# yunjinli/visual-slam

Hardware: AMD Instinct MI355X
Metric: stereo frames/sec, detect+describe (1500 feats) + stereo match, 752x480 (higher is better)
Workload: dtype u8/f32/f64; 1 GPU; synthetic 752x480 stereo, 1500 feats/frame (BASELINE configs[1]); independent streams per GPU (configs[3]); inputs_resident_in_hbm=True, distinct_stereo_pairs_per_gpu=1024, distinct_scenes_per_gpu=64, stereo_frames_per_pass_per_gpu=1024, hip_streams=2, stereo_frames_per_launch=512, num_features=1500, match=threshold 70, ratio 1.2, cross-check

## Files before the change

### include/vslam_hip.h

```cpp
#ifndef VSLAM_HIP_H
#define VSLAM_HIP_H

#include <stddef.h>
#include <stdint.h>

#ifdef __cplusplus
extern "C" {
#endif

#define VSL_OK 0
#define VSL_ERR_INVALID (-1)
#define VSL_ERR_HIP (-2)
#define VSL_ERR_NOMEM (-3)
#define VSL_ERR_CAPACITY (-4)
#define VSL_ERR_NO_DEVICE (-5)
#define VSL_ERR_IO (-6)
#define VSL_ERR_NUMERIC (-7)

typedef struct vsl_ctx vsl_ctx;


const char* vsl_version(void);
const char* vsl_last_error(const vsl_ctx* ctx);
int vsl_device_count(void);
// ... 74 lines not shown
int vsl_frames_upload(vsl_ctx* ctx, vsl_frames* f, int first, int n, const uint8_t* imgs,
                      size_t pitch, size_t img_stride);
int vsl_host_register(vsl_ctx* ctx, void* ptr, size_t bytes);
int vsl_host_unregister(vsl_ctx* ctx, void* ptr);
int vsl_frames_detect_describe(vsl_ctx* ctx, vsl_frames* f, int first, int n, int num_features,
                               int rotate_features);
int vsl_frames_resolve_ties(vsl_ctx* ctx, vsl_frames* f, int* n_resolved);
int vsl_frames_exact_fallbacks(const vsl_frames* f);
int vsl_ctx_set_tie_eps(vsl_ctx* ctx, double eps);
int vsl_ctx_set_diagnostic(vsl_ctx* ctx, const char* name, int value);
int vsl_ctx_get_diagnostic(vsl_ctx* ctx, const char* name, int* value);

int vsl_frames_match(vsl_ctx* ctx, vsl_frames* f, const int32_t* slot_pairs, int n_pairs,
                     int threshold, double dist_2_best);
int vsl_frames_download_keypoints(vsl_ctx* ctx, vsl_frames* f, int slot, int cap,
                                  double* corners_xy, double* angles, uint64_t* desc, int* n_out);
int vsl_frames_download_matches(vsl_ctx* ctx, vsl_frames* f, int pair, int cap_pairs,
                                int32_t* pairs, int* n_out);
int vsl_frames_download_counts(vsl_ctx* ctx, vsl_frames* f, int n_images, int32_t* n_keypoints,
                               int n_pairs, int32_t* n_matches);

int vsl_frames_stereo_inliers(vsl_ctx* ctx, vsl_frames* f, int first_pair, int n_pairs, int model_a, const double* intr8_a,
                              int model_b, const double* intr8_b, const double* E9, const double* R9_0_1,
                              const double* t3_0_1, double threshold, int triangulate);
int vsl_frames_download_inliers(vsl_ctx* ctx, vsl_frames* f, int pair, int cap_pairs, int32_t* pairs, double* points_c,
                                int* n_out);
int vsl_frames_download_inlier_counts(vsl_ctx* ctx, vsl_frames* f, int n_pairs, int32_t* counts);
int vsl_find_inliers_essential(vsl_ctx* ctx, int model_a, const double* intr8_a, int model_b, const double* intr8_b,
                               const double* E9, const double* kp_a_xy, int n_a, const double* kp_b_xy, int n_b,
                               const int32_t* matches, int n_matches, double threshold, const double* R9_0_1,
                               const double* t3_0_1, int32_t* pairs_out, double* points_out, int* n_out);

int vsl_frames_download_candidate_counts(vsl_ctx* ctx, vsl_frames* f, int n_images, int32_t* n_candidates);

int vsl_diag_sqrt_check(vsl_ctx* ctx, uint32_t lo_bits, uint32_t hi_bits, unsigned long long* n_mismatch);

int vsl_diag_frames_describe_at(vsl_ctx* ctx, vsl_frames* f, int first, int n, const int32_t* corners_xy,
                                const int32_t* counts, int cap, int rotate_features, int32_t* moments,
                                int32_t* tie_rec, int tie_rec_cap, int* n_ties);

int vsl_diag_frames_set_keypoints(vsl_ctx* ctx, vsl_frames* f, int first, int n, const int32_t* counts, int cap,
                                  const int32_t* corners_xy, const uint64_t* desc);

int vsl_map_create(vsl_ctx* ctx, int cap_landmarks, int cap_descriptors, vsl_map** out);
void vsl_map_destroy(vsl_map* map);
int vsl_map_append_descriptors(vsl_map* map, int n, const uint64_t* desc, int* first_index);
int vsl_map_append_descriptors_from_frame(vsl_map* map, vsl_frames* f, int slot, int n, const int32_t* feature_ids,
                                          int* first_index);
int vsl_map_set_landmarks(vsl_map* map, int n, const double* points, const int32_t* obs_start,
                          const int32_t* obs_pool_index);
int vsl_map_info(const vsl_map* map, int* n_landmarks, int* n_observation_refs, int* n_descriptors);
int vsl_map_track(vsl_map* map, vsl_frames* f, int slot, const double* pose7, int cam_model, const double* intr8, int width,
                  int height, double cam_z_threshold, double match_max_dist_2d, int feature_match_threshold,
                  double feature_match_dist_2_best, int32_t* pairs, int* n_pairs, int* n_projected);
int vsl_map_track_corners(vsl_map* map, vsl_frames* f, int slot, const double* pose7, int cam_model, const double* intr8,
                          int width, int height, double cam_z_threshold, double match_max_dist_2d, int feature_match_threshold,
                          double feature_match_dist_2_best, int32_t* pairs, int* n_pairs, int* n_projected, double* corners_xy,
                          int* n_corners);

enum { VSL_CAM_DS = 0, VSL_CAM_PINHOLE = 1, VSL_CAM_EUCM = 2, VSL_CAM_KB4 = 3 };

typedef struct vsl_ba_problem {
  int32_t n_cams;
  int32_t n_lms;
  int32_t n_obs;
  int32_t cam_model[2];
// ... 202 lines not shown
```

### visual-slam_amd/__init__.py

```python
import ctypes as C
import os
from pathlib import Path

import numpy as np

_DIR = Path(__file__).resolve().parent
_SO = _DIR / "libvslam_hip.so"
_LIB = None

u8p = C.POINTER(C.c_uint8)
i32p = C.POINTER(C.c_int32)
u32p = C.POINTER(C.c_uint32)
u64p = C.POINTER(C.c_uint64)
i64p = C.POINTER(C.c_int64)
f32p = C.POINTER(C.c_float)
f64p = C.POINTER(C.c_double)

STAGES = ["response", "select", "describe", "match", "match_finalize", "ba_linearize", "ba_schur",
          "ba_solve", "bow_transform", "bow_score", "ba_finish", "ba_step"]

SPD_PATHS = ["none", "dense_panels", "band_panels", "band_fused", "band_two_ended", "bcr", "bcr_cyclic"]

OK = 0
CAM_DS, CAM_PINHOLE, CAM_EUCM, CAM_KB4 = 0, 1, 2, 3
# ... 1070 lines not shown

    def bow_vectors(self, first, n, voc, num_features=1500, levelsup=4, db=None, cap_per_image=None, host_outputs=True):
        L, ctx = self.ctx.L, self.ctx
        n = int(n)
        cap = (2 * num_features + 512 if cap_per_image is None else int(cap_per_image)) if host_outputs else 0
        nfeat = np.zeros(max(n, 1), np.int32)
        index = np.zeros(max(n, 1), np.int32)
        for attempt in range(2):
            m = max(n * cap, 1)
            ids, vals = np.zeros(m, np.uint32), np.zeros(m, np.float64)
            fn, ff = np.zeros(m, np.uint32), np.zeros(m, np.uint32)
            nnz, fvn = np.zeros(max(n, 1), np.int32), np.zeros(max(n, 1), np.int32)
            rc = L.vsl_frames_bow_vectors(ctx.h, self.h, int(first), n, voc.h if voc is not None else None, int(num_features),
                                          int(levelsup), db.h if db is not None else None, index.ctypes.data_as(i32p), cap,
                                          ids.ctypes.data_as(u32p), vals.ctypes.data_as(f64p), nnz.ctypes.data_as(i32p),
                                          fn.ctypes.data_as(u32p), ff.ctypes.data_as(u32p), fvn.ctypes.data_as(i32p),
                                          nfeat.ctypes.data_as(i32p))
            if rc != -4 or cap == 0 or cap_per_image is not None or nfeat[:n].max(initial=0) <= cap:
                break
            cap = int(nfeat[:n].max())
        ctx._ck(rc)
        out = None
        if host_outputs:
            out = [(ids[i * cap:i * cap + nnz[i]].copy(), vals[i * cap:i * cap + nnz[i]].copy(),
                    fn[i * cap:i * cap + fvn[i]].copy(), ff[i * cap:i * cap + fvn[i]].copy()) for i in range(n)]
        return (out, index[:n].copy()) if db is not None else out

    def candidate_counts(self, n_images):
        nc = np.zeros(max(n_images, 1), np.int32)
        self.ctx._ck(self.ctx.L.vsl_frames_download_candidate_counts(self.ctx.h, self.h, int(n_images),
                                                                     nc.ctypes.data_as(i32p)))
        return nc[:n_images].copy()

    def counts(self, n_images, n_pairs):
        nk = np.zeros(max(n_images, 1), np.int32)
        nm = np.zeros(max(n_pairs, 1), np.int32)
        self.ctx._ck(self.ctx.L.vsl_frames_download_counts(self.ctx.h, self.h, int(n_images),
                                                           nk.ctypes.data_as(i32p), int(n_pairs),
                                                           nm.ctypes.data_as(i32p)))
        return nk[:n_images].copy(), nm[:n_pairs].copy()


class Map:

    def __init__(self, ctx, cap_landmarks=4096, cap_descriptors=16384):
        self.ctx = ctx
        hnd = C.c_void_p()
        ctx._ck(ctx.L.vsl_map_create(ctx.h, int(cap_landmarks), int(cap_descriptors), C.byref(hnd)))
        self.h = hnd

    def close(self):
        if getattr(self, "h", None):
            self.ctx.L.vsl_map_destroy(self.h)
            self.h = None

    def __del__(self):
        try:
            self.close()
        except Exception:
            pass

    def append_descriptors(self, desc):
        desc = np.ascontiguousarray(desc, np.uint64).reshape(-1, 4)
        first = C.c_int32()
        self.ctx._ck(self.ctx.L.vsl_map_append_descriptors(self.h, len(desc), desc.ctypes.data_as(u64p), C.byref(first)))
        return first.value
# ... 41 lines not shown
```

### visual-slam_amd/csrc/ctx.hip

```cpp
#include <cmath>

#include "vsl_common.h"

static thread_local char g_noctx_err[512] = "";

int vsl_fail(vsl_ctx* ctx, int code, const char* fmt, ...) {
  char* dst = ctx ? ctx->err : g_noctx_err;
  va_list ap;
  va_start(ap, fmt);
  vsnprintf(dst, 512, fmt, ap);
  va_end(ap);
  return code;
}

extern "C" const char* vsl_version(void) { return "vslam_hip 0.1 (gfx950)"; }

extern "C" const char* vsl_last_error(const vsl_ctx* ctx) { return ctx ? ctx->err : g_noctx_err; }

extern "C" int vsl_device_count(void) {
  int n = 0;
  if (hipGetDeviceCount(&n) != hipSuccess) return 0;
  return n;
}

// ... 376 lines not shown
    int rc = vsl_frames_alloc(ctx, 2, w, h, feat, 1, &ctx->scratch);
    if (rc) return rc;
    ctx->scratch_w = w;
    ctx->scratch_h = h;
    ctx->scratch_feat = feat;
  }
  *out = ctx->scratch;
  return VSL_OK;
}

extern "C" int vsl_frames_download_counts(vsl_ctx* ctx, vsl_frames* f, int n_images, int32_t* n_keypoints,
                                          int n_pairs, int32_t* n_matches) {
  if (!ctx || !f || n_images < 0 || n_images > f->max_images || n_pairs < 0 || n_pairs > f->max_pairs)
    return vsl_fail(ctx, VSL_ERR_INVALID, "vsl_frames_download_counts: bad arguments");
  if (n_images > 0 && n_keypoints)
    VSL_HIP(ctx, hipMemcpyAsync(n_keypoints, f->kp_count, sizeof(int32_t) * n_images, hipMemcpyDeviceToHost, ctx->stream));
  if (n_pairs > 0 && n_matches)
    VSL_HIP(ctx, hipMemcpyAsync(n_matches, f->match_count, sizeof(int32_t) * n_pairs, hipMemcpyDeviceToHost, ctx->stream));
  VSL_HIP(ctx, hipStreamSynchronize(ctx->stream));
  return VSL_OK;
}

extern "C" int vsl_frames_download_candidate_counts(vsl_ctx* ctx, vsl_frames* f, int n_images, int32_t* n_candidates) {
  if (!ctx || !f || n_images < 0 || n_images > f->max_images || !n_candidates)
    return vsl_fail(ctx, VSL_ERR_INVALID, "vsl_frames_download_candidate_counts: bad arguments");
  if (n_images == 0) return VSL_OK;
  std::vector<int32_t> m((size_t)n_images * VSL_META_STRIDE);
  VSL_HIP(ctx, hipMemcpyAsync(m.data(), f->meta, sizeof(int32_t) * m.size(), hipMemcpyDeviceToHost, ctx->stream));
  VSL_HIP(ctx, hipStreamSynchronize(ctx->stream));
  for (int i = 0; i < n_images; i++) n_candidates[i] = m[(size_t)i * VSL_META_STRIDE + VSL_META_NCAND_LAST];
  return VSL_OK;
}

extern "C" int vsl_frames_download_keypoints(vsl_ctx* ctx, vsl_frames* f, int slot, int cap, double* corners_xy,
                                             double* angles, uint64_t* desc, int* n_out) {
  if (!ctx || !f || slot < 0 || slot >= f->max_images || !n_out || cap < 0)
    return vsl_fail(ctx, VSL_ERR_INVALID, "vsl_frames_download_keypoints: bad arguments");
  const size_t F = (size_t)f->F;
  void* hp = nullptr;
  int rc = vsl_ctx_hpinned(ctx, 64 + F * (8 + 8 + 32), &hp);
  if (rc) return rc;
  int32_t* hdr = (int32_t*)hp;
  int32_t* hxy = (int32_t*)((char*)hp + 64);
  int32_t* hmom = hxy + 2 * F;
  uint64_t* hdesc = (uint64_t*)(hmom + 2 * F);
  const size_t base = (size_t)slot * F;
  const bool ties = f->ties_pending;
  hdr[0] = 0;
  if (ties) VSL_HIP(ctx, hipMemcpyAsync(&hdr[0], f->tie_count, sizeof(int32_t), hipMemcpyDeviceToHost, ctx->stream));
  VSL_HIP(ctx, hipMemcpyAsync(&hdr[1], f->kp_count + slot, sizeof(int32_t), hipMemcpyDeviceToHost, ctx->stream));
  VSL_HIP(ctx, hipMemcpyAsync(hxy, f->kp_xy + base * 2, sizeof(int32_t) * 2 * F, hipMemcpyDeviceToHost, ctx->stream));
  if (angles) VSL_HIP(ctx, hipMemcpyAsync(hmom, f->kp_moments + base * 2, sizeof(int32_t) * 2 * F, hipMemcpyDeviceToHost, ctx->stream));
  if (desc) VSL_HIP(ctx, hipMemcpyAsync(hdesc, f->kp_desc + base * 4, sizeof(uint64_t) * 4 * F, hipMemcpyDeviceToHost, ctx->stream));
  VSL_HIP(ctx, hipStreamSynchronize(ctx->stream));
  if (ties) {
    if (hdr[0] != 0) {
      if ((rc = vsl_resolve_ties(ctx, f, nullptr))) return rc;
      if (desc) {
        VSL_HIP(ctx, hipMemcpyAsync(hdesc, f->kp_desc + base * 4, sizeof(uint64_t) * 4 * F, hipMemcpyDeviceToHost, ctx->stream));
        VSL_HIP(ctx, hipStreamSynchronize(ctx->stream));
      }
    } else {
      f->ties_settled();
    }
  }
  const int n = hdr[1];
// ... 59 lines not shown
```

### visual-slam_amd/csrc/detect.hip

```cpp
#include <type_traits>

#include "vsl_common.h"

#ifndef K1_ROWS
#define K1_ROWS 60
#endif
#ifndef K1_ROWS_SMALL
#define K1_ROWS_SMALL 29
#endif
#define VSL_QUALITY_LEVEL 0.01
#define K1_WLIST 384
#define K1_COLS 60

__device__ __forceinline__ int reflect101(int i, int n) { return i < 0 ? -i : (i >= n ? 2 * n - 2 - i : i); }

struct RowF {
  float rx, ry;
};

struct RowRaw {
  unsigned l, m, r;
};

typedef __amdgpu_buffer_rsrc_t ImgSrd;
__device__ __forceinline__ RowRaw rowload(ImgSrd img, int w, int yr, unsigned xm, unsigned xe, unsigned xp) {
  const int row = yr * w;
  RowRaw o;
  o.l = __builtin_amdgcn_raw_buffer_load_b8(img, (int)xm, row, 0);
  o.m = __builtin_amdgcn_raw_buffer_load_b8(img, (int)xe, row, 0);
  o.r = __builtin_amdgcn_raw_buffer_load_b8(img, (int)xp, row, 0);
  return o;
}

__device__ __forceinline__ RowF rowfilt(RowRaw p, float s, float s2) {
  const float l = (float)p.l, m = (float)p.m, r = (float)p.r;
  RowF o;
  o.rx = r - l;
  float t = s * l;
  t = t + s2 * m;
  t = t + s * r;
  o.ry = t;
  return o;
}

// ... 39 lines not shown
}
__device__ __forceinline__ float sqrt_rn(float t) {
  float r = fast_sqrt_rn(t);
  const bool small = t < K1_SQRT_FLOOR;
  if (__builtin_amdgcn_ballot_w64(small) != 0ull) {
    asm volatile("" ::: "memory");
    const bool rare = small && t > 0.f;
    if (__builtin_amdgcn_ballot_w64(rare) != 0ull) {
      asm volatile("" ::: "memory");
      if (rare) r = sqrtf(t);
    }
  }
  return r;
}

__global__ void sqrt_check_kernel(uint32_t lo, uint32_t hi, unsigned long long* bad) {
  const uint64_t stride = (uint64_t)gridDim.x * blockDim.x;
  unsigned long long n = 0;
  for (uint64_t b = (uint64_t)lo + blockIdx.x * blockDim.x + threadIdx.x; b <= hi; b += stride) {
    const float t = __builtin_bit_cast(float, (uint32_t)b);
    n += __builtin_bit_cast(uint32_t, fast_sqrt_rn(t)) != __builtin_bit_cast(uint32_t, sqrtf(t));
  }
  if (n) atomicAdd(bad, n);
}

__global__ void detect_init_kernel(int32_t* meta, int first, int n) {
  const int i = blockIdx.x * blockDim.x + threadIdx.x;
  if (i < n) {
    meta[(size_t)(first + i) * VSL_META_STRIDE + VSL_META_MAX] = INT32_MIN;
    meta[(size_t)(first + i) * VSL_META_STRIDE + VSL_META_NCAND] = 0;
  }
}

template <bool STORE_RESPONSE, int ROWS>
__global__ __launch_bounds__(256) void min_eig_response_kernel(const uint8_t* __restrict__ images,
                                                               float* __restrict__ response, int32_t* __restrict__ meta,
                                                               uint64_t* __restrict__ cand, size_t cand_cap, int w, int h,
                                                               int first, int wlist_cap, int n_images, int tiles_x, int tiles_y) {
  __shared__ uint64_t list[4][K1_WLIST];
  __shared__ int wave_n[4], wave_max[4], g_base;
  __shared__ double xbuf[4][2][66];
  const int tiles = tiles_x * tiles_y;
  int img_i, tile;
  if (n_images >= 8) {
    const int xcd = blockIdx.x & 7, sl = blockIdx.x >> 3;
    img_i = (sl / tiles) * 8 + xcd;
    tile = sl - (sl / tiles) * tiles;
  } else {
    img_i = blockIdx.x / tiles;
    tile = blockIdx.x - img_i * tiles;
  }
  if (img_i >= n_images) return;
  const int bx = tile % tiles_x, by = tile / tiles_x;
  const int slot = first + img_i;
  const ImgSrd img = __builtin_amdgcn_make_buffer_rsrc((void*)(images + (size_t)slot * w * h), 0, w * h, 0x00020000);
  float* __restrict__ resp = response + (size_t)slot * w * h;
  const int lane = threadIdx.x & 63;
  const int wave = __builtin_amdgcn_readfirstlane(threadIdx.x >> 6);
  const int xs = bx * K1_COLS;
  const int y0 = (by * 4 + wave) * ROWS;
  int n_wave = 0;
  int own_max = INT32_MIN;
  if (y0 < h) {
    const float s = (float)(1.0 / (4.0 * 3.0 * 255.0));
    const float s2 = 2.0f * s;
    const int x = xs - 2 + lane;
    const unsigned xe = (unsigned)reflect101(min(max(x, -1), w), w);
    const unsigned xm = (unsigned)reflect101((int)xe - 1, w), xp = (unsigned)reflect101((int)xe + 1, w);
    const bool own_col = lane >= 2 && lane < 2 + K1_COLS && x < w;
    const bool cand_col = own_col && x >= 1 && x < w - 1;
    const unsigned long long cand_lanes = __builtin_amdgcn_ballot_w64(cand_col);

    struct R3 {
      double xx, xy, yy;
    };
    R3 ra = {0, 0, 0}, rb = ra, bs = ra;
    float va = 0.f, vb = 0.f, hA = 0.f, hB = 0.f, hC = 0.f;
    RowF fA = {0.f, 0.f}, fB = fA, fC = fA;
    int prev_ye = -100, pre_row = -100;
    RowRaw pre = {0u, 0u, 0u};
    float vmax = -3.0e38f;
    const int y_end = min(h, y0 + ROWS);
    auto step = [&](auto steady_tag, auto even_tag, int q, R3& r2, R3& r1, float& v_mid_slot, float& v_dn_slot, float& h_up,
                    float& h_mid, float& h_dn, RowF& f0, RowF& f1, RowF& f2) {
      constexpr bool STEADY = decltype(steady_tag)::value;
      constexpr bool EVEN = decltype(even_tag)::value;
      if (STEADY) {
        f2 = rowfilt(pre, s, s2);
        pre = rowload(img, w, min(q + 2, h - 1), xm, xe, xp);
      } else {
        const int ye = reflect101(min(max(q, -1), h), h);
        if (ye == prev_ye + 1 && ye + 1 < h) {
          if (pre_row != ye + 1) pre = rowload(img, w, ye + 1, xm, xe, xp);
          f2 = rowfilt(pre, s, s2);
        } else {
          f0 = rowfilt(rowload(img, w, reflect101(ye - 1, h), xm, xe, xp), s, s2);
          f1 = rowfilt(rowload(img, w, ye, xm, xe, xp), s, s2);
          f2 = rowfilt(rowload(img, w, reflect101(ye + 1, h), xm, xe, xp), s, s2);
        }
        pre_row = min(ye + 2, h - 1);
        pre = rowload(img, w, pre_row, xm, xe, xp);
        prev_ye = ye;
      }
      const float dx = (f0.rx + f2.rx) * s + f1.rx * s2;
// ... 6 lines not shown
        asm volatile("" ::: "memory");
        const double lxx = xbuf[wave][0][lane], uxx = xbuf[wave][0][lane + 2];
        const double lxy = xbuf[wave][1][lane], uxy = xbuf[wave][1][lane + 2];
        asm volatile("" ::: "memory");
        cur.xx = (lxx + dxx) + uxx;
        cur.xy = (lxy + dxy) + uxy;
        cur.yy = (dpp_below_f64(dyy) + dyy) + dpp_above_f64(dyy);
      }
      const int y = q - 1;
      double Axx, Axy, Ayy;
      if (EVEN) {
        bs.xx = r1.xx + cur.xx;
        bs.xy = r1.xy + cur.xy;
        bs.yy = r1.yy + cur.yy;
        Axx = r2.xx + bs.xx;
        Axy = r2.xy + bs.xy;
        Ayy = r2.yy + bs.yy;
      } else {
        Axx = bs.xx + cur.xx;
        Axy = bs.xy + cur.xy;
        Ayy = bs.yy + cur.yy;
      }
      r2 = cur;
      const float X = (float)Axx, b = (float)Axy, Y = (float)Ayy;
      const float xpy = X + Y, d = 0.5f * (X - Y);
      float t = d * d;
      t = t + b * b;
      const float v_dn = __builtin_fmaf(0.5f, xpy, -sqrt_rn(t));
      float h_tmp;
      asm volatile("s_nop 1\n\tv_max_f32_dpp %0, %2, %2 wave_shr:1 row_mask:0xf bank_mask:0xf bound_ctrl:0\n\t"
                   "v_max_f32_dpp %1, %2, %0 wave_shl:1 row_mask:0xf bank_mask:0xf bound_ctrl:0"
                   : "=&v"(h_tmp), "=&v"(h_dn)
                   : "v"(v_dn));
      if (own_col && y >= y0 && y < y_end) {
        if (STORE_RESPONSE) resp[y * w + x] = v_dn;
        vmax = fmax2(vmax, v_dn);
      }
      const float v_mid = v_mid_slot;
      const int yc = q - 2;
      if (yc >= y0 && yc < y_end && yc >= 1 && yc < h - 1) {
        const float m9 = fmax3(h_up, h_mid, h_dn);
        const bool ge0 = v_mid >= m9;
        if ((__builtin_amdgcn_ballot_w64(ge0) & cand_lanes) != 0ull) {
          const bool ge = ge0 && v_mid > 0.f;
          const unsigned long long mask = __builtin_amdgcn_ballot_w64(ge) & cand_lanes;
          if (cand_col && ge) {
            const uint32_t ob = (uint32_t)vsl_float_to_ordered(v_mid) ^ 0x80000000u;
            const uint64_t key = ((uint64_t)ob << 32) | ((uint32_t)yc << 16) | (uint32_t)x;
            const int p = n_wave + (int)__builtin_amdgcn_mbcnt_hi((uint32_t)(mask >> 32),
                                                                  __builtin_amdgcn_mbcnt_lo((uint32_t)mask, 0u));
            if (__builtin_expect(p < wlist_cap, 1)) {
              list[wave][p] = key;
            } else {
              const int g = atomicAdd(&meta[(size_t)slot * VSL_META_STRIDE + VSL_META_NCAND], 1);
              if ((size_t)g < cand_cap) cand[(size_t)slot * cand_cap + g] = key;
            }
          }
          n_wave += __popcll(mask);
        }
      }
      v_dn_slot = v_dn;
    };
    const int q_first = y0 - 2, q_last = y_end + 1;
    typedef std::integral_constant<bool, true> Steady;
    typedef std::integral_constant<bool, false> Generic;
    typedef std::integral_constant<bool, true> Even;
    typedef std::integral_constant<bool, false> Odd;
#define K1_STEP_E0(T, q) step(T{}, Even{}, q, ra, rb, va, vb, hA, hB, hC, fA, fB, fC)
#define K1_STEP_O1(T, q) step(T{}, Odd{}, q, rb, ra, vb, va, hB, hC, hA, fB, fC, fA)
#define K1_STEP_E2(T, q) step(T{}, Even{}, q, ra, rb, va, vb, hC, hA, hB, fC, fA, fB)
#define K1_STEP_O3(T, q) step(T{}, Odd{}, q, rb, ra, vb, va, hA, hB, hC, fA, fB, fC)
#define K1_STEP_E4(T, q) step(T{}, Even{}, q, ra, rb, va, vb, hB, hC, hA, fB, fC, fA)
#define K1_STEP_O5(T, q) step(T{}, Odd{}, q, rb, ra, vb, va, hC, hA, hB, fC, fA, fB)
    constexpr int K1_OPEN = (ROWS + 4) % 6;
    static_assert(K1_OPEN == 3 || K1_OPEN == 4, "opening sequence written for 3 or 4 steps");
#define K1_STRIP(T)                                \
  K1_STEP_E0(Generic, q_first);                    \
  K1_STEP_O1(T, q_first + 1);                      \
  K1_STEP_E2(T, q_first + 2);                      \
  if constexpr (K1_OPEN == 3) {                    \
    for (int q = q_first + 3; q <= q_last; q += 6) { \
      K1_STEP_O3(T, q);                            \
      K1_STEP_E4(T, q + 1);                        \
      K1_STEP_O5(T, q + 2);                        \
      K1_STEP_E0(T, q + 3);                        \
      K1_STEP_O1(T, q + 4);                        \
      K1_STEP_E2(T, q + 5);                        \
    }                                              \
  } else {                                         \
    K1_STEP_O3(T, q_first + 3);                    \
    for (int q = q_first + 4; q <= q_last; q += 6) { \
      K1_STEP_E4(T, q);                            \
      K1_STEP_O5(T, q + 1);                        \
      K1_STEP_E0(T, q + 2);                        \
      K1_STEP_O1(T, q + 3);                        \
      K1_STEP_E2(T, q + 4);                        \
      K1_STEP_O3(T, q + 5);                        \
    }                                              \
  }
    if (q_first >= 1 && q_last + 1 < h) {
      K1_STRIP(Steady)
    } else {
      K1_STRIP(Generic)
    }
#undef K1_STRIP
#undef K1_STEP_E0
#undef K1_STEP_O1
#undef K1_STEP_E2
#undef K1_STEP_O3
#undef K1_STEP_E4
#undef K1_STEP_O5
#pragma unroll
    for (int o = 32; o > 0; o >>= 1) vmax = fmaxf(vmax, __shfl_xor(vmax, o));
    own_max = vsl_float_to_ordered(vmax);
    if (lane == 0) atomicMax(&meta[(size_t)slot * VSL_META_STRIDE + VSL_META_MAX], own_max);
  }
  if (lane == 0) wave_max[wave] = own_max;
  __syncthreads();
  int kept = min(n_wave, wlist_cap);
  {
    const float wg_max = vsl_ordered_to_float(max(max(wave_max[0], wave_max[1]), max(wave_max[2], wave_max[3])));
    if (wg_max > 0.f && kept > 0) {
      const float thr = (float)((double)wg_max * VSL_QUALITY_LEVEL);
      const uint32_t floor_hi = (uint32_t)vsl_float_to_ordered(thr) ^ 0x80000000u;
      const int have = kept;
      kept = 0;
      for (int i0 = 0; i0 < have; i0 += 64) {
        const int i = i0 + lane;
        const uint64_t key = i < have ? list[wave][i] : 0ull;
        const bool keep = i < have && (uint32_t)(key >> 32) > floor_hi;
        const unsigned long long m = __builtin_amdgcn_ballot_w64(keep);
        if (keep) list[wave][kept + (int)__builtin_amdgcn_mbcnt_hi((uint32_t)(m >> 32), __builtin_amdgcn_mbcnt_lo((uint32_t)m, 0u))] = key;
        kept += __popcll(m);
      }
    }
  }
  if (lane == 0) wave_n[wave] = kept;
  __syncthreads();
  const int c0 = wave_n[0], c1 = wave_n[1], c2 = wave_n[2], c3 = wave_n[3];
  const int n = c0 + c1 + c2 + c3;
  if (n == 0) return;
  if (threadIdx.x == 0) g_base = atomicAdd(&meta[(size_t)slot * VSL_META_STRIDE + VSL_META_NCAND], n);
  __syncthreads();
  const int base = g_base + (wave > 0 ? c0 : 0) + (wave > 1 ? c1 : 0) + (wave > 2 ? c2 : 0);
  const int mine = wave_n[wave];
  for (int i = lane; i < mine; i += 64)
    if ((size_t)(base + i) < cand_cap) cand[(size_t)slot * cand_cap + base + i] = list[wave][i];
}

#define SEL_THREADS 1024
#define SEL_CHUNK 8192
#define SEL_BINS 1024
#define SEL_MAX_BLOCKERS 6
static_assert(SEL_THREADS <= 1024 && SEL_MAX_BLOCKERS * 10 <= 64, "blocker packing");

struct SelShared {
  int wave_tot[16];
  int hist[256];
  unsigned long long sel_prefix;
  int sel_k;
  int n_chunk;
};

__device__ __forceinline__ int block_scan(bool p, bool q, int* wave_tot, int& total) {
  const int lane = threadIdx.x & 63, wave = __builtin_amdgcn_readfirstlane(threadIdx.x >> 6);
  const unsigned long long m = __ballot(p), mq = __ballot(q);
  const int within = (int)__builtin_amdgcn_mbcnt_hi((uint32_t)(m >> 32), __builtin_amdgcn_mbcnt_lo((uint32_t)m, 0u)) |
                     (int)__builtin_amdgcn_mbcnt_hi((uint32_t)(mq >> 32), __builtin_amdgcn_mbcnt_lo((uint32_t)mq, 0u)) << 16;
  const int mine = __popcll(m) | __popcll(mq) << 16;
  if (lane == 0) wave_tot[wave] = mine;
  __syncthreads();
  int x = wave_tot[lane & 15];
  x += __builtin_amdgcn_update_dpp(0, x, 0x111, 0xf, 0xf, true);
  x += __builtin_amdgcn_update_dpp(0, x, 0x112, 0xf, 0xf, true);
  x += __builtin_amdgcn_update_dpp(0, x, 0x114, 0xf, 0xf, true);
  x += __builtin_amdgcn_update_dpp(0, x, 0x118, 0xf, 0xf, true);
  total = __builtin_amdgcn_readlane(x, 15);
  return __builtin_amdgcn_readlane(x, wave) - mine + within;
}

// ... 411 lines not shown
          if (ns) {
            __hip_atomic_store(&state[tid], ns, __ATOMIC_RELAXED, __HIP_MEMORY_SCOPE_WORKGROUP);
            undecided = false;
            accepted = ns == 1;
          }
        }
        __builtin_amdgcn_s_sleep(1);
      }
      const bool inside = px >= border && px < w - border && py >= border && py < h - border;
      int total = 0;
      const int pre = block_scan(accepted, accepted && inside, sh->wave_tot, total);
      const int lim = num_features - n_acc;
      const bool cut = (total & 0xFFFF) > lim;
      const bool keep = accepted && (pre & 0xFFFF) < lim;
      const bool inb = keep && inside;
      if (inb) {
        const int pos = n_out + (pre >> 16);
        out[2 * pos] = px;
        out[2 * pos + 1] = py;
      }
      if (cut && accepted && (pre & 0xFFFF) == lim) sh->sel_k = pre >> 16;
      if (keep) sel_acc_insert(acc, cell, SEL_ACC_VALID | (uint32_t)((py & 7) << 3) | (uint32_t)(px & 7));
      if (alive) head[cell] = (uint16_t)SEL_HEAD_EMPTY;
      n_acc = min(num_features, n_acc + (total & 0xFFFF));
      __syncthreads();
      n_out += cut ? sh->sel_k : total >> 16;
    }
    hi = lo;
    remaining -= n_chunk;
  }
  if (tid == 0) {
    kp_count[slot] = n_out;
    meta[(size_t)slot * VSL_META_STRIDE + VSL_META_NCAND_LAST] = n_cand_raw;
    meta[(size_t)slot * VSL_META_STRIDE + VSL_META_MAX] = INT32_MIN;
    meta[(size_t)slot * VSL_META_STRIDE + VSL_META_NCAND] = 0;
  }
}

extern "C" int vsl_diag_sqrt_check(vsl_ctx* ctx, uint32_t lo_bits, uint32_t hi_bits, unsigned long long* n_mismatch) {
  if (!ctx || !n_mismatch || lo_bits > hi_bits || hi_bits > 0x7f7fffffu)
    return vsl_fail(ctx, VSL_ERR_INVALID, "vsl_diag_sqrt_check: bad range");
  VSL_HIP(ctx, hipSetDevice(ctx->device));
  void* d = nullptr;
  int rc = vsl_ctx_dscratch(ctx, sizeof(unsigned long long), &d);
  if (rc) return rc;
  VSL_HIP(ctx, hipMemsetAsync(d, 0, sizeof(unsigned long long), ctx->stream));
  hipLaunchKernelGGL(sqrt_check_kernel, dim3(4096), dim3(256), 0, ctx->stream, lo_bits, hi_bits, (unsigned long long*)d);
  VSL_CHECK_LAUNCH(ctx);
  VSL_HIP(ctx, hipMemcpyAsync(n_mismatch, d, sizeof(unsigned long long), hipMemcpyDeviceToHost, ctx->stream));
  VSL_HIP(ctx, hipStreamSynchronize(ctx->stream));
  return VSL_OK;
}

int vsl_launch_detect(vsl_ctx* ctx, vsl_frames* f, int first, int n, int num_features) {
  if (n <= 0) return VSL_OK;
  if (num_features < 1 || num_features > f->F)
    return vsl_fail(ctx, VSL_ERR_INVALID, "num_features %d not in [1, %d]", num_features, f->F);
  static_assert(sizeof(SelShared) <= 2048, "SelShared fits its LDS slot");
  const int cells = (((f->w + 7) / 8 + 2) * ((f->h + 7) / 8 + 2) + 1) & ~1;
  const bool grid_global = cells > SEL_MAX_CELLS;
  if (grid_global && !f->sel_grid) {
    VSL_HIP(ctx, hipMalloc((void**)&f->sel_grid, sizeof(uint32_t) * (size_t)cells * f->max_images));
  }
  const int w = f->w, h = f->h;
  {
    VslStage st(ctx, VSL_STAGE_RESPONSE);
    if (f->detect_meta_dirty)
      hipLaunchKernelGGL(detect_init_kernel, dim3((f->max_images + 255) / 256), dim3(256), 0, ctx->stream, f->meta, 0, f->max_images);
    f->detect_meta_dirty = true;
    const bool small = n < 8 && !f->store_response;
    const int rows = small ? K1_ROWS_SMALL : K1_ROWS;
    const int tiles_y = (h + 4 * rows - 1) / (4 * rows);
    const int tiles_x = (w + K1_COLS - 1) / K1_COLS;
    const dim3 k1_grid((unsigned)(tiles_x * tiles_y) * (unsigned)(n >= 8 ? 8 * ((n + 7) / 8) : n));
    const int wcap = ctx->k1_list_cap < 0 ? K1_WLIST : min(ctx->k1_list_cap, K1_WLIST);
    if (f->store_response)
      hipLaunchKernelGGL((min_eig_response_kernel<true, K1_ROWS>), k1_grid, dim3(256), 0, ctx->stream, f->images, f->response, f->meta,
                         f->cand, f->cand_cap, w, h, first, wcap, n, tiles_x, tiles_y);
    else if (small)
      hipLaunchKernelGGL((min_eig_response_kernel<false, K1_ROWS_SMALL>), k1_grid, dim3(256), 0, ctx->stream, f->images, f->response, f->meta,
                         f->cand, f->cand_cap, w, h, first, wcap, n, tiles_x, tiles_y);
    else
      hipLaunchKernelGGL((min_eig_response_kernel<false, K1_ROWS>), k1_grid, dim3(256), 0, ctx->stream, f->images, f->response, f->meta,
                         f->cand, f->cand_cap, w, h, first, wcap, n, tiles_x, tiles_y);
    VSL_CHECK_LAUNCH(ctx);
  }
  {
    VslStage st(ctx, VSL_STAGE_SELECT);
    if (grid_global)
      hipLaunchKernelGGL(select_kernel<true>, dim3(n), dim3(SEL_THREADS), 0, ctx->stream, f->cand, f->meta, f->kp_xy,
                         f->kp_count, w, h, f->cand_cap, f->F, first, num_features, 19, VSL_QUALITY_LEVEL, f->sel_grid, ctx->select_bucket_cap);
    else
      hipLaunchKernelGGL(select_kernel<false>, dim3(n), dim3(SEL_THREADS), 0, ctx->stream, f->cand, f->meta, f->kp_xy,
                         f->kp_count, w, h, f->cand_cap, f->F, first, num_features, 19, VSL_QUALITY_LEVEL, (uint32_t*)nullptr,
                         ctx->select_bucket_cap);
    VSL_CHECK_LAUNCH(ctx);
  }
  f->detect_meta_dirty = false;
  return VSL_OK;
}
```

### visual-slam_amd/csrc/vsl_common.h

```cpp
#pragma once
#include <hip/hip_runtime.h>

#include <chrono>
#include <cstdarg>
#include <cstdint>
#include <cstdio>
#include <cstring>
#include <string>
#include <vector>

#include "../../include/vslam_hip.h"
#include "chol_plan.h"

#define VSL_WAVE 64
#define VSL_META_STRIDE 32
#define VSL_META_MAX 0
#define VSL_META_NCAND 1
#define VSL_META_NEXACT 3
#define VSL_META_NCAND_LAST 4
#define VSL_META_NEXACT_LAST 5
#define VSL_EXACT_CAP 16384
#ifndef VSL_TILE_LX
#define VSL_TILE_LX 7
#endif
#ifndef VSL_TILE_LY
#define VSL_TILE_LY 7
#endif
#define VSL_TIE_OVERFLOW_FLAG 0x40000000u

inline double now_ms() {
  return std::chrono::duration<double, std::milli>(std::chrono::steady_clock::now().time_since_epoch()).count();
}

struct vsl_ctx {
  int device = 0;
  hipStream_t stream = nullptr;
  bool owns_stream = false;
  char err[512] = {0};
  bool profiling = false;
  struct StageEv {
    hipEvent_t a, b;
    int stage;
  };
  std::vector<StageEv> pending;
  std::vector<hipEvent_t> ev_pool;
  double stage_ms[VSL_STAGE_COUNT] = {0};
  int64_t stage_launches[VSL_STAGE_COUNT] = {0};
  struct vsl_frames* scratch = nullptr;
  int scratch_w = 0, scratch_h = 0, scratch_feat = 0;
  void* dscratch = nullptr;
  size_t dscratch_cap = 0;
  void* hpinned = nullptr;
  size_t hpinned_cap = 0;
// ... 213 lines not shown
```

Baseline: 385,800 frames/s.

## Remap response kernel to column-major strips with taller rows and early list flushing

The min-eigenvalue response kernel now gives each wave its own strip, indexed column-major, with 120 rows per strip instead of 60, so less halo is recomputed per pixel. The candidate list is flushed to global memory partway through a strip whenever it nears capacity, using a wave-local quality cut. The max used for that cut is now tracked only from candidate pixels and edge pixels instead of every owned pixel. The kernel also records the per-image max response in meta, with a new download API and Python wrapper to read it. The risks are fewer blocks for small batches and a wave-local quality threshold that differs from the workgroup-wide one, which could keep a different set of candidates.

```diff
diff --git a/include/vslam_hip.h b/include/vslam_hip.h
--- a/include/vslam_hip.h
+++ b/include/vslam_hip.h
@@ -130,6 +130,7 @@
                                const double* t3_0_1, int32_t* pairs_out, double* points_out, int* n_out);
 
 int vsl_frames_download_candidate_counts(vsl_ctx* ctx, vsl_frames* f, int n_images, int32_t* n_candidates);
+int vsl_frames_download_response_max(vsl_ctx* ctx, vsl_frames* f, int n_images, float* response_max);
 
 int vsl_diag_sqrt_check(vsl_ctx* ctx, uint32_t lo_bits, uint32_t hi_bits, unsigned long long* n_mismatch);
 
diff --git a/visual-slam_amd/__init__.py b/visual-slam_amd/__init__.py
--- a/visual-slam_amd/__init__.py
+++ b/visual-slam_amd/__init__.py
@@ -1126,6 +1126,12 @@
                                                                      nc.ctypes.data_as(i32p)))
         return nc[:n_images].copy()
 
+    def response_max(self, n_images):
+        mx = np.zeros(max(n_images, 1), np.float32)
+        self.ctx._ck(self.ctx.L.vsl_frames_download_response_max(self.ctx.h, self.h, int(n_images),
+                                                                 mx.ctypes.data_as(C.POINTER(C.c_float))))
+        return mx[:n_images].copy()
+
     def counts(self, n_images, n_pairs):
         nk = np.zeros(max(n_images, 1), np.int32)
         nm = np.zeros(max(n_pairs, 1), np.int32)
diff --git a/visual-slam_amd/csrc/ctx.hip b/visual-slam_amd/csrc/ctx.hip
--- a/visual-slam_amd/csrc/ctx.hip
+++ b/visual-slam_amd/csrc/ctx.hip
@@ -432,6 +432,17 @@
   return VSL_OK;
 }
 
+extern "C" int vsl_frames_download_response_max(vsl_ctx* ctx, vsl_frames* f, int n_images, float* response_max) {
+  if (!ctx || !f || n_images < 0 || n_images > f->max_images || !response_max)
+    return vsl_fail(ctx, VSL_ERR_INVALID, "vsl_frames_download_response_max: bad arguments");
+  if (n_images == 0) return VSL_OK;
+  std::vector<int32_t> m((size_t)n_images * VSL_META_STRIDE);
+  VSL_HIP(ctx, hipMemcpyAsync(m.data(), f->meta, sizeof(int32_t) * m.size(), hipMemcpyDeviceToHost, ctx->stream));
+  VSL_HIP(ctx, hipStreamSynchronize(ctx->stream));
+  for (int i = 0; i < n_images; i++) response_max[i] = vsl_ordered_to_float(m[(size_t)i * VSL_META_STRIDE + VSL_META_MAX_LAST]);
+  return VSL_OK;
+}
+
 extern "C" int vsl_frames_download_keypoints(vsl_ctx* ctx, vsl_frames* f, int slot, int cap, double* corners_xy,
                                              double* angles, uint64_t* desc, int* n_out) {
   if (!ctx || !f || slot < 0 || slot >= f->max_images || !n_out || cap < 0)
diff --git a/visual-slam_amd/csrc/detect.hip b/visual-slam_amd/csrc/detect.hip
--- a/visual-slam_amd/csrc/detect.hip
+++ b/visual-slam_amd/csrc/detect.hip
@@ -3,13 +3,14 @@
 #include "vsl_common.h"
 
 #ifndef K1_ROWS
-#define K1_ROWS 60
+#define K1_ROWS 120
 #endif
 #ifndef K1_ROWS_SMALL
-#define K1_ROWS_SMALL 29
+#define K1_ROWS_SMALL 30
 #endif
 #define VSL_QUALITY_LEVEL 0.01
 #define K1_WLIST 384
+#define K1_FLUSH_ROOM 96
 #define K1_COLS 60
 
 __device__ __forceinline__ int reflect101(int i, int n) { return i < 0 ? -i : (i >= n ? 2 * n - 2 - i : i); }
@@ -115,15 +116,33 @@
   }
 }
 
+
+__device__ __forceinline__ int k1_quality_cut(uint64_t* list, int have, float vmax, int lane) {
+  if (!(vmax > 0.f) || have <= 0) return have;
+  const float thr = (float)((double)vmax * VSL_QUALITY_LEVEL);
+  const uint32_t floor_hi = (uint32_t)vsl_float_to_ordered(thr) ^ 0x80000000u;
+  int kept = 0;
+  for (int i0 = 0; i0 < have; i0 += 64) {
+    const int i = i0 + lane;
+    const uint64_t key = i < have ? list[i] : 0ull;
+    const bool keep = i < have && (uint32_t)(key >> 32) > floor_hi;
+    const unsigned long long m = __builtin_amdgcn_ballot_w64(keep);
+    if (keep) list[kept + (int)__builtin_amdgcn_mbcnt_hi((uint32_t)(m >> 32), __builtin_amdgcn_mbcnt_lo((uint32_t)m, 0u))] = key;
+    kept += __popcll(m);
+  }
+  return kept;
+}
+
 template <bool STORE_RESPONSE, int ROWS>
 __global__ __launch_bounds__(256) void min_eig_response_kernel(const uint8_t* __restrict__ images,
                                                                float* __restrict__ response, int32_t* __restrict__ meta,
                                                                uint64_t* __restrict__ cand, size_t cand_cap, int w, int h,
-                                                               int first, int wlist_cap, int n_images, int tiles_x, int tiles_y) {
+                                                               int first, int wlist_cap, int n_images, int tiles_x, int strips_y) {
   __shared__ uint64_t list[4][K1_WLIST];
   __shared__ int wave_n[4], wave_max[4], g_base;
   __shared__ double xbuf[4][2][66];
-  const int tiles = tiles_x * tiles_y;
+  const int strips = tiles_x * strips_y;
+  const int tiles = (strips + 3) >> 2;
   int img_i, tile;
   if (n_images >= 8) {
     const int xcd = blockIdx.x & 7, sl = blockIdx.x >> 3;
@@ -134,17 +153,20 @@
     tile = blockIdx.x - img_i * tiles;
   }
   if (img_i >= n_images) return;
-  const int bx = tile % tiles_x, by = tile / tiles_x;
   const int slot = first + img_i;
   const ImgSrd img = __builtin_amdgcn_make_buffer_rsrc((void*)(images + (size_t)slot * w * h), 0, w * h, 0x00020000);
   float* __restrict__ resp = response + (size_t)slot * w * h;
   const int lane = threadIdx.x & 63;
   const int wave = __builtin_amdgcn_readfirstlane(threadIdx.x >> 6);
+  const int strip = tile * 4 + wave;
+  const int bx = strip / strips_y;
   const int xs = bx * K1_COLS;
-  const int y0 = (by * 4 + wave) * ROWS;
+  const int y0 = (strip - bx * strips_y) * ROWS;
+  int* const ncand = &meta[(size_t)slot * VSL_META_STRIDE + VSL_META_NCAND];
+  uint64_t* const cand_img = cand + (size_t)slot * cand_cap;
   int n_wave = 0;
   int own_max = INT32_MIN;
-  if (y0 < h) {
+  if (strip < strips) {
     const float s = (float)(1.0 / (4.0 * 3.0 * 255.0));
     const float s2 = 2.0f * s;
     const int x = xs - 2 + lane;
@@ -153,6 +175,8 @@
     const bool own_col = lane >= 2 && lane < 2 + K1_COLS && x < w;
     const bool cand_col = own_col && x >= 1 && x < w - 1;
     const unsigned long long cand_lanes = __builtin_amdgcn_ballot_w64(cand_col);
+    const bool edge_strip = xs == 0 || xs + K1_COLS >= w;
+    const bool edge_lane = own_col && (x == 0 || x == w - 1);
 
     struct R3 {
       double xx, xy, yy;
@@ -225,9 +249,12 @@
                    "v_max_f32_dpp %1, %2, %0 wave_shl:1 row_mask:0xf bank_mask:0xf bound_ctrl:0"
                    : "=&v"(h_tmp), "=&v"(h_dn)
                    : "v"(v_dn));
-      if (own_col && y >= y0 && y < y_end) {
-        if (STORE_RESPONSE) resp[y * w + x] = v_dn;
-        vmax = fmax2(vmax, v_dn);
+      if (STORE_RESPONSE) {
+        if (own_col && y >= y0 && y < y_end) resp[y * w + x] = v_dn;
+      }
+      const bool edge_row = !STEADY && (y == 0 || y == h - 1);
+      if ((edge_strip || edge_row) && y >= y0 && y < y_end) {
+        if (edge_row ? own_col : edge_lane) vmax = fmax2(vmax, v_dn);
       }
       const float v_mid = v_mid_slot;
       const int yc = q - 2;
@@ -238,6 +265,7 @@
           const bool ge = ge0 && v_mid > 0.f;
           const unsigned long long mask = __builtin_amdgcn_ballot_w64(ge) & cand_lanes;
           if (cand_col && ge) {
+            vmax = fmax2(vmax, v_mid);
             const uint32_t ob = (uint32_t)vsl_float_to_ordered(v_mid) ^ 0x80000000u;
             const uint64_t key = ((uint64_t)ob << 32) | ((uint32_t)yc << 16) | (uint32_t)x;
             const int p = n_wave + (int)__builtin_amdgcn_mbcnt_hi((uint32_t)(mask >> 32),
@@ -245,14 +273,28 @@
             if (__builtin_expect(p < wlist_cap, 1)) {
               list[wave][p] = key;
             } else {
-              const int g = atomicAdd(&meta[(size_t)slot * VSL_META_STRIDE + VSL_META_NCAND], 1);
-              if ((size_t)g < cand_cap) cand[(size_t)slot * cand_cap + g] = key;
+              const int g = atomicAdd(ncand, 1);
+              if ((size_t)g < cand_cap) cand_img[g] = key;
             }
           }
           n_wave += __popcll(mask);
         }
       }
       v_dn_slot = v_dn;
+    };
+    auto flush = [&]() {
+      float m = vmax;
+#pragma unroll
+      for (int o = 32; o > 0; o >>= 1) m = fmaxf(m, __shfl_xor(m, o));
+      const int kept = k1_quality_cut(list[wave], min(n_wave, wlist_cap), m, lane);
+      if (kept > 0) {
+        int g = 0;
+        if (lane == 0) g = atomicAdd(ncand, kept);
+        g = __builtin_amdgcn_readfirstlane(g);
+        for (int i = lane; i < kept; i += 64)
+          if ((size_t)(g + i) < cand_cap) cand_img[g + i] = list[wave][i];
+      }
+      n_wave = 0;
     };
     const int q_first = y0 - 2, q_last = y_end + 1;
     typedef std::integral_constant<bool, true> Steady;
@@ -265,38 +307,52 @@
 #define K1_STEP_O3(T, q) step(T{}, Odd{}, q, rb, ra, vb, va, hA, hB, hC, fA, fB, fC)
 #define K1_STEP_E4(T, q) step(T{}, Even{}, q, ra, rb, va, vb, hB, hC, hA, fB, fC, fA)
 #define K1_STEP_O5(T, q) step(T{}, Odd{}, q, rb, ra, vb, va, hC, hA, hB, fC, fA, fB)
-    constexpr int K1_OPEN = (ROWS + 4) % 6;
-    static_assert(K1_OPEN == 3 || K1_OPEN == 4, "opening sequence written for 3 or 4 steps");
-#define K1_STRIP(T)                                \
-  K1_STEP_E0(Generic, q_first);                    \
-  K1_STEP_O1(T, q_first + 1);                      \
-  K1_STEP_E2(T, q_first + 2);                      \
-  if constexpr (K1_OPEN == 3) {                    \
-    for (int q = q_first + 3; q <= q_last; q += 6) { \
-      K1_STEP_O3(T, q);                            \
-      K1_STEP_E4(T, q + 1);                        \
-      K1_STEP_O5(T, q + 2);                        \
-      K1_STEP_E0(T, q + 3);                        \
-      K1_STEP_O1(T, q + 4);                        \
-      K1_STEP_E2(T, q + 5);                        \
-    }                                              \
-  } else {                                         \
-    K1_STEP_O3(T, q_first + 3);                    \
-    for (int q = q_first + 4; q <= q_last; q += 6) { \
-      K1_STEP_E4(T, q);                            \
-      K1_STEP_O5(T, q + 1);                        \
-      K1_STEP_E0(T, q + 2);                        \
-      K1_STEP_O1(T, q + 3);                        \
-      K1_STEP_E2(T, q + 4);                        \
-      K1_STEP_O3(T, q + 5);                        \
-    }                                              \
-  }
-    if (q_first >= 1 && q_last + 1 < h) {
-      K1_STRIP(Steady)
+#define K1_STEP_R(r, T, q)                            \
+  do {                                                \
+    if constexpr ((r) % 6 == 0) K1_STEP_E0(T, q);      \
+    else if constexpr ((r) % 6 == 1) K1_STEP_O1(T, q); \
+    else if constexpr ((r) % 6 == 2) K1_STEP_E2(T, q); \
+    else if constexpr ((r) % 6 == 3) K1_STEP_O3(T, q); \
+    else if constexpr ((r) % 6 == 4) K1_STEP_E4(T, q); \
+    else K1_STEP_O5(T, q);                            \
+  } while (0)
+    constexpr int K1_OPEN = ROWS % 6 + 4;
+#define K1_OPENING(T)                                          \
+  K1_STEP_R(1, T, q_first + 1);                                \
+  K1_STEP_R(2, T, q_first + 2);                                \
+  K1_STEP_R(3, T, q_first + 3);                                \
+  if constexpr (K1_OPEN > 4) K1_STEP_R(4, T, q_first + 4);     \
+  if constexpr (K1_OPEN > 5) K1_STEP_R(5, T, q_first + 5);     \
+  if constexpr (K1_OPEN > 6) K1_STEP_R(6, T, q_first + 6);     \
+  if constexpr (K1_OPEN > 7) K1_STEP_R(7, T, q_first + 7);     \
+  if constexpr (K1_OPEN > 8) K1_STEP_R(8, T, q_first + 8);
+#define K1_SIX(T, q)               \
+  K1_STEP_R(K1_OPEN, T, q);        \
+  K1_STEP_R(K1_OPEN + 1, T, q + 1); \
+  K1_STEP_R(K1_OPEN + 2, T, q + 2); \
+  K1_STEP_R(K1_OPEN + 3, T, q + 3); \
+  K1_STEP_R(K1_OPEN + 4, T, q + 4); \
+  K1_STEP_R(K1_OPEN + 5, T, q + 5);
+    K1_STEP_E0(Generic, q_first);
+    if (q_first >= 1 && q_first + K1_OPEN < h) {
+      K1_OPENING(Steady)
     } else {
-      K1_STRIP(Generic)
-    }
-#undef K1_STRIP
+      K1_OPENING(Generic)
+    }
+    const int flush_mark = max(wlist_cap - K1_FLUSH_ROOM, 0);
+    int q = q_first + K1_OPEN;
+    for (; q <= q_last && q + 6 < h; q += 6) {
+      K1_SIX(Steady, q)
+      if (n_wave > flush_mark) flush();
+    }
+    prev_ye = q - 1;
+    pre_row = min(q + 1, h - 1);
+    for (; q <= q_last; q += 6) {
+      K1_SIX(Generic, q)
+    }
+#undef K1_STEP_R
+#undef K1_OPENING
+#undef K1_SIX
 #undef K1_STEP_E0
 #undef K1_STEP_O1
 #undef K1_STEP_E2
@@ -310,35 +366,19 @@
   }
   if (lane == 0) wave_max[wave] = own_max;
   __syncthreads();
-  int kept = min(n_wave, wlist_cap);
-  {
-    const float wg_max = vsl_ordered_to_float(max(max(wave_max[0], wave_max[1]), max(wave_max[2], wave_max[3])));
-    if (wg_max > 0.f && kept > 0) {
-      const float thr = (float)((double)wg_max * VSL_QUALITY_LEVEL);
-      const uint32_t floor_hi = (uint32_t)vsl_float_to_ordered(thr) ^ 0x80000000u;
-      const int have = kept;
-      kept = 0;
-      for (int i0 = 0; i0 < have; i0 += 64) {
-        const int i = i0 + lane;
-        const uint64_t key = i < have ? list[wave][i] : 0ull;
-        const bool keep = i < have && (uint32_t)(key >> 32) > floor_hi;
-        const unsigned long long m = __builtin_amdgcn_ballot_w64(keep);
-        if (keep) list[wave][kept + (int)__builtin_amdgcn_mbcnt_hi((uint32_t)(m >> 32), __builtin_amdgcn_mbcnt_lo((uint32_t)m, 0u))] = key;
-        kept += __popcll(m);
-      }
-    }
-  }
+  const float wg_max = vsl_ordered_to_float(max(max(wave_max[0], wave_max[1]), max(wave_max[2], wave_max[3])));
+  const int kept = k1_quality_cut(list[wave], min(n_wave, wlist_cap), wg_max, lane);
   if (lane == 0) wave_n[wave] = kept;
   __syncthreads();
   const int c0 = wave_n[0], c1 = wave_n[1], c2 = wave_n[2], c3 = wave_n[3];
   const int n = c0 + c1 + c2 + c3;
   if (n == 0) return;
-  if (threadIdx.x == 0) g_base = atomicAdd(&meta[(size_t)slot * VSL_META_STRIDE + VSL_META_NCAND], n);
+  if (threadIdx.x == 0) g_base = atomicAdd(ncand, n);
   __syncthreads();
   const int base = g_base + (wave > 0 ? c0 : 0) + (wave > 1 ? c1 : 0) + (wave > 2 ? c2 : 0);
   const int mine = wave_n[wave];
   for (int i = lane; i < mine; i += 64)
-    if ((size_t)(base + i) < cand_cap) cand[(size_t)slot * cand_cap + base + i] = list[wave][i];
+    if ((size_t)(base + i) < cand_cap) cand_img[base + i] = list[wave][i];
 }
 
 #define SEL_THREADS 1024
@@ -816,6 +856,7 @@
   if (tid == 0) {
     kp_count[slot] = n_out;
     meta[(size_t)slot * VSL_META_STRIDE + VSL_META_NCAND_LAST] = n_cand_raw;
+    meta[(size_t)slot * VSL_META_STRIDE + VSL_META_MAX_LAST] = vsl_float_to_ordered(maxv);
     meta[(size_t)slot * VSL_META_STRIDE + VSL_META_MAX] = INT32_MIN;
     meta[(size_t)slot * VSL_META_STRIDE + VSL_META_NCAND] = 0;
   }
@@ -854,19 +895,19 @@
     f->detect_meta_dirty = true;
     const bool small = n < 8 && !f->store_response;
     const int rows = small ? K1_ROWS_SMALL : K1_ROWS;
-    const int tiles_y = (h + 4 * rows - 1) / (4 * rows);
+    const int strips_y = (h + rows - 1) / rows;
     const int tiles_x = (w + K1_COLS - 1) / K1_COLS;
-    const dim3 k1_grid((unsigned)(tiles_x * tiles_y) * (unsigned)(n >= 8 ? 8 * ((n + 7) / 8) : n));
+    const dim3 k1_grid((unsigned)((tiles_x * strips_y + 3) / 4) * (unsigned)(n >= 8 ? 8 * ((n + 7) / 8) : n));
     const int wcap = ctx->k1_list_cap < 0 ? K1_WLIST : min(ctx->k1_list_cap, K1_WLIST);
     if (f->store_response)
       hipLaunchKernelGGL((min_eig_response_kernel<true, K1_ROWS>), k1_grid, dim3(256), 0, ctx->stream, f->images, f->response, f->meta,
-                         f->cand, f->cand_cap, w, h, first, wcap, n, tiles_x, tiles_y);
+                         f->cand, f->cand_cap, w, h, first, wcap, n, tiles_x, strips_y);
     else if (small)
       hipLaunchKernelGGL((min_eig_response_kernel<false, K1_ROWS_SMALL>), k1_grid, dim3(256), 0, ctx->stream, f->images, f->response, f->meta,
-                         f->cand, f->cand_cap, w, h, first, wcap, n, tiles_x, tiles_y);
+                         f->cand, f->cand_cap, w, h, first, wcap, n, tiles_x, strips_y);
     else
       hipLaunchKernelGGL((min_eig_response_kernel<false, K1_ROWS>), k1_grid, dim3(256), 0, ctx->stream, f->images, f->response, f->meta,
-                         f->cand, f->cand_cap, w, h, first, wcap, n, tiles_x, tiles_y);
+                         f->cand, f->cand_cap, w, h, first, wcap, n, tiles_x, strips_y);
     VSL_CHECK_LAUNCH(ctx);
   }
   {
diff --git a/visual-slam_amd/csrc/vsl_common.h b/visual-slam_amd/csrc/vsl_common.h
--- a/visual-slam_amd/csrc/vsl_common.h
+++ b/visual-slam_amd/csrc/vsl_common.h
@@ -19,6 +19,7 @@
 #define VSL_META_NEXACT 3
 #define VSL_META_NCAND_LAST 4
 #define VSL_META_NEXACT_LAST 5
+#define VSL_META_MAX_LAST 6
 #define VSL_EXACT_CAP 16384
 #ifndef VSL_TILE_LX
 #define VSL_TILE_LX 7
```

Measured after the change: 398,000 frames/s (median of 6 runs). 1.03x the previous value.
